# LingmaFuture/PRCV2025REID

Measured on AMD Instinct MI355X. Metric: multimodal instances/sec (PxK, 5-modality) at 1/2/4/8 GPU; eval queries/sec, higher is better.
Workload: dtype bf16; 1 GPU; P=16,K=4 per GPU, vis/nir/sk/cp 224x224 + text (T<=77), CLIP ViT-B/16 + text tower random-init, MER-LoRA r=8, masks all-on, 400 ids, SDM+CE, fwd+bwd+grad sanitise/clip+AdamW (reference default trainable set); P=16, K=4, global_batch=64, lora_rank=8, accum_steps=1, parallelism=dp1

## Files before the change

prcv2025reid_amd/csrc/attention.hip:

```cpp
#include "common.h"
#include <stdlib.h>

namespace {

typedef __attribute__((ext_vector_type(4))) short s4;
typedef __attribute__((address_space(3))) s4* lds_s4_ptr;

constexpr float LOG2E = 1.4426950408889634f;

__device__ __forceinline__ int swz(int row, int c) { return c ^ ((row >> 1) & 7); }

typedef const __attribute__((address_space(1))) void* gptr_t;
typedef __attribute__((address_space(3))) void* lptr_t;

template <int NT>
__device__ __forceinline__ void stage_head(const bf16_t* __restrict__ base, int ld, int S, char* lds, int wave, int lane,
                                           int row_limit = 1 << 30) {
#pragma unroll
    for (int i = 0; i < 4; ++i) {
        const int rblk = (i * NT + wave) * 8;
        if (rblk >= row_limit) continue;
        const int row = rblk + (lane >> 3);
        const int c = swz(row, lane & 7);
        const int grow = row < S ? row : S - 1;
        __builtin_amdgcn_global_load_lds((gptr_t)(base + (size_t)grow * ld + c * 8), (lptr_t)(lds + rblk * 128), 16, 0, 0);
    }
}

__device__ __forceinline__ bf16x8 row_frag(const char* img, int row0, int kchunk, int lane) {
    const int row = row0 + (lane & 31);
    return *(const bf16x8*)(img + row * 128 + (swz(row, kchunk + (lane >> 5)) << 4));
}

__device__ __forceinline__ bf16x8 col_frag(const char* img, int krow0, int col0, int lane) {
    const int h = lane >> 5, half16 = (lane >> 4) & 1, i = lane & 15;
    const int q = i >> 2, pp = i & 3;
    const int col = col0 + 16 * half16 + 4 * pp;
    const int r_lo = krow0 + 4 * h + q, r_hi = r_lo + 8;
    const char* a_lo = img + r_lo * 128 + (swz(r_lo, col >> 3) << 4) + (col & 7) * 2;
    const char* a_hi = img + r_hi * 128 + (swz(r_hi, col >> 3) << 4) + (col & 7) * 2;
    const s4 lo = __builtin_amdgcn_ds_read_tr16_b64_v4i16((lds_s4_ptr)a_lo);
    const s4 hi = __builtin_amdgcn_ds_read_tr16_b64_v4i16((lds_s4_ptr)a_hi);
    return bf16x8{lo[0], lo[1], lo[2], lo[3], hi[0], hi[1], hi[2], hi[3]};
}

__device__ __forceinline__ bf16x8 gfrag(const bf16_t* __restrict__ base, int ld, int row, int kchunk, int lane) {
    return *(const bf16x8*)(base + (size_t)row * ld + (kchunk + (lane >> 5)) * 8);
}

struct FragOff {
    int row[4];
    int col_lo[2];
    int col_hi[2];
};
__device__ __forceinline__ FragOff make_frag_off(int lane) {
    FragOff f;
    const int r = lane & 31, h = lane >> 5;
#pragma unroll
    for (int ks = 0; ks < 4; ++ks) f.row[ks] = r * 128 + (swz(r, 2 * ks + h) << 4);
    const int half16 = (lane >> 4) & 1, i = lane & 15, q = i >> 2, pp = i & 3;
    const int r_lo = 4 * h + q, r_hi = r_lo + 8;
#pragma unroll
    for (int dt = 0; dt < 2; ++dt) {
        const int col = dt * 32 + 16 * half16 + 4 * pp;
        f.col_lo[dt] = r_lo * 128 + (swz(r_lo, col >> 3) << 4) + (col & 7) * 2;
        f.col_hi[dt] = r_hi * 128 + (swz(r_hi, col >> 3) << 4) + (col & 7) * 2;
    }
    return f;
}
__device__ __forceinline__ bf16x8 row_frag_o(const char* img, int tile_row0, int ks, const FragOff& f) {
    return *(const bf16x8*)(img + tile_row0 * 128 + f.row[ks]);
}
__device__ __forceinline__ bf16x8 col_frag_o(const char* img, int krow0, int dt, const FragOff& f) {
    const s4 lo = __builtin_amdgcn_ds_read_tr16_b64_v4i16((lds_s4_ptr)(img + krow0 * 128 + f.col_lo[dt]));
    const s4 hi = __builtin_amdgcn_ds_read_tr16_b64_v4i16((lds_s4_ptr)(img + krow0 * 128 + f.col_hi[dt]));
    return bf16x8{lo[0], lo[1], lo[2], lo[3], hi[0], hi[1], hi[2], hi[3]};
}
__device__ __forceinline__ float fast_exp2(float x) { return __builtin_amdgcn_exp2f(x); }

__device__ __forceinline__ bf16x8 pack8(const f32x16& a, int s) {
    bf16x8 r;
#pragma unroll
    for (int j = 0; j < 8; ++j) r[j] = (short)f32_to_bf16(a[8 * s + j]);
    return r;
}

__device__ __forceinline__ int acc_row(int reg, int lane) { return (reg & 3) + 8 * (reg >> 2) + 4 * (lane >> 5); }

struct AttnParams {
    const bf16_t* qkv; int ld; const uint8_t* key_mask;
    bf16_t* out; int ldo; float* lse;
    const bf16_t* dout; bf16_t* dqkv; int lddqkv; float* delta;
    int n_seq, S, heads, causal;
    int q_tiles;
};

__device__ __forceinline__ void store_tile_row16(bf16_t* row, bool ok, const f32x16& t, float scale, int lane) {
#pragma unroll
    for (int j = 0; j < 2; ++j) {
        const int a = 8 * j, b = 8 * j + 4;
        const auto r0 = __builtin_amdgcn_permlane32_swap(pack_bf16x2(t[a] * scale, t[a + 1] * scale),
                                                         pack_bf16x2(t[b] * scale, t[b + 1] * scale), false, false);
        const auto r1 = __builtin_amdgcn_permlane32_swap(pack_bf16x2(t[a + 2] * scale, t[a + 3] * scale),
                                                         pack_bf16x2(t[b + 2] * scale, t[b + 3] * scale), false, false);
        if (ok) *(uint4*)(row + 8 * (2 * j + (lane >> 5))) = uint4{r0[0], r1[0], r0[1], r1[1]};
    }
}


template <int NT, bool TWO_PASS>
__global__ __launch_bounds__(NT * 64, TWO_PASS ? 4 : 1) void attn_fwd_kernel(const AttnParams p) {
    REID_T16_ENTER();
    extern __shared__ __attribute__((aligned(16))) char smem[];
    char* Ks = smem;
    char* Vs = smem + NT * 32 * 128;
    const int tid = threadIdx.x, lane = tid & 63;
    const int wave = __builtin_amdgcn_readfirstlane(tid >> 6);
    const int seq = blockIdx.x / p.heads, head = blockIdx.x % p.heads;
    const int d = p.heads * 64;
    const bf16_t* qb = p.qkv + (size_t)seq * p.S * p.ld + head * 64;
    stage_head<NT>(qb + d, p.ld, p.S, Ks, wave, lane);
    const int q0 = wave * 32;
    const int qi = q0 + (lane & 31);
    const int qrow = qi < p.S ? qi : p.S - 1;
    bf16x8 qf[4];
#pragma unroll
    for (int ks = 0; ks < 4; ++ks) qf[ks] = gfrag(qb, p.ld, qrow, 2 * ks, lane);
    stage_head<NT>(qb + 2 * d, p.ld, p.S, Vs, wave, lane);
    __syncthreads();
    if (q0 >= p.S || (p.q_tiles > 0 && wave >= p.q_tiles)) return;

    const FragOff fo = make_frag_off(lane);
    const uint8_t* km = p.key_mask ? p.key_mask + (size_t)seq * p.S : nullptr;
    const int h4 = 4 * (lane >> 5);
    const bool general = km != nullptr || p.causal;
    auto score_tile = [&](int kt) -> f32x16 {
        f32x16 t;
#pragma unroll
        for (int e = 0; e < 16; ++e) t[e] = 0.f;
#pragma unroll
        for (int ks = 0; ks < 4; ++ks) t = mfma32(row_frag_o(Ks, kt * 32, ks, fo), qf[ks], t);
        if (general) {
#pragma unroll
            for (int e = 0; e < 16; ++e) {
                const int key = kt * 32 + (e & 3) + 8 * (e >> 2) + h4;
                bool ok = key < p.S;
                if (ok && km) ok = km[key] != 0;
                if (p.causal) ok = ok && key <= qi;
                t[e] = ok ? t[e] : -INFINITY;
            }
        } else if (kt == NT - 1) {
#pragma unroll
            for (int e = 0; e < 16; ++e) {
                const int key = kt * 32 + (e & 3) + 8 * (e >> 2) + h4;
                t[e] = key < p.S ? t[e] : -INFINITY;
            }
        }
        return t;
    };
    const float c = 0.125f * LOG2E;
    f32x16 ot[2];
#pragma unroll
    for (int dt = 0; dt < 2; ++dt)
#pragma unroll
        for (int e = 0; e < 16; ++e) ot[dt][e] = 0.f;
    float mx = -INFINITY, l = 0.f;
    if (TWO_PASS) {
#pragma unroll 1
        for (int kt = 0; kt < NT; ++kt) {
            const f32x16 t = score_tile(kt);
#pragma unroll
            for (int e = 0; e < 16; e += 2) mx = fmaxf(mx, fmaxf(t[e], t[e + 1]));
        }
        mx = fmaxf(mx, __shfl_xor(mx, 32, 64));
        if (mx == -INFINITY) mx = 0.f;
        const float nmc = -mx * c;
#pragma unroll 1
        for (int kt = 0; kt < NT; ++kt) {
            f32x16 t = score_tile(kt);
#pragma unroll
            for (int e = 0; e < 16; ++e) {
                const float pe = fast_exp2(fmaf(t[e], c, nmc));
                t[e] = pe;
                l += pe;
            }
#pragma unroll
            for (int s2 = 0; s2 < 2; ++s2) {
                const bf16x8 pf = pack8(t, s2);
#pragma unroll
                for (int dt = 0; dt < 2; ++dt) ot[dt] = mfma32(col_frag_o(Vs, kt * 32 + 16 * s2, dt, fo), pf, ot[dt]);
            }
        }
    } else {
        f32x16 st[NT];
#pragma unroll
        for (int kt = 0; kt < NT; ++kt) st[kt] = score_tile(kt);
#pragma unroll
        for (int kt = 0; kt < NT; ++kt)
#pragma unroll
            for (int e = 0; e < 16; e += 2) mx = fmaxf(mx, fmaxf(st[kt][e], st[kt][e + 1]));
        mx = fmaxf(mx, __shfl_xor(mx, 32, 64));
        if (mx == -INFINITY) mx = 0.f;
        const float nmc = -mx * c;
#pragma unroll
        for (int kt = 0; kt < NT; ++kt)
#pragma unroll
            for (int e = 0; e < 16; ++e) {
                const float pe = fast_exp2(fmaf(st[kt][e], c, nmc));
                st[kt][e] = pe;
                l += pe;
            }
#pragma unroll
        for (int kt = 0; kt < NT; ++kt)
#pragma unroll
            for (int s2 = 0; s2 < 2; ++s2) {
                const bf16x8 pf = pack8(st[kt], s2);
#pragma unroll
                for (int dt = 0; dt < 2; ++dt) ot[dt] = mfma32(col_frag_o(Vs, kt * 32 + 16 * s2, dt, fo), pf, ot[dt]);
            }
    }
    l += __shfl_xor(l, 32, 64);
    {
        const float inv = 1.0f / l;
        bf16_t* orow = p.out + ((size_t)seq * p.S + qrow) * p.ldo + head * 64;
#pragma unroll
        for (int dt = 0; dt < 2; ++dt) store_tile_row16(orow + dt * 32, qi < p.S, ot[dt], inv, lane);
        if (qi < p.S && p.lse && lane < 32) p.lse[((size_t)seq * p.heads + head) * p.S + qi] = mx * 0.125f + logf(l);
    }
}

template <int NT>
__global__ __launch_bounds__(NT * 64) void attn_bwd_dkv_kernel(const AttnParams p) {
    REID_T16_ENTER();
    extern __shared__ __attribute__((aligned(16))) char smem[];
    char* Qs = smem;
    char* Gs = smem + NT * 32 * 128;
    float* rowc = (float*)(smem + 2 * NT * 32 * 128);
    const int tid = threadIdx.x, lane = tid & 63;
    const int wave = __builtin_amdgcn_readfirstlane(tid >> 6);
    const int seq = blockIdx.x / p.heads, head = blockIdx.x % p.heads;
    const int d = p.heads * 64;
    const bf16_t* qb = p.qkv + (size_t)seq * p.S * p.ld + head * 64;
    const bf16_t* gb = p.dout + (size_t)seq * p.S * p.ldo + head * 64;
    const int q_rows = p.q_tiles > 0 ? p.q_tiles * 32 : NT * 32;
    stage_head<NT>(qb, p.ld, p.S, Qs, wave, lane, q_rows);
    stage_head<NT>(gb, p.ldo, p.S, Gs, wave, lane, q_rows);
    for (int t = tid; t < NT * 32; t += NT * 64) {
        const size_t o = ((size_t)seq * p.heads + head) * p.S + t;
        rowc[t] = t < p.S ? -p.lse[o] * LOG2E : -INFINITY;
        rowc[NT * 32 + t] = t < p.S ? -p.delta[o] * 0.125f : 0.f;
    }
    const int k0 = wave * 32;
    const int ki = k0 + (lane & 31);
    const int krow = ki < p.S ? ki : p.S - 1;
    bf16x8 kf[4], vf[4];
#pragma unroll
    for (int ks = 0; ks < 4; ++ks) {
        kf[ks] = gfrag(qb + d, p.ld, krow, 2 * ks, lane);
        vf[ks] = gfrag(qb + 2 * d, p.ld, krow, 2 * ks, lane);
    }
    __syncthreads();
    if (k0 >= p.S) return;
    const uint8_t* km = p.key_mask ? p.key_mask + (size_t)seq * p.S : nullptr;
    const bool key_ok = ki < p.S && (!km || km[ki] != 0);

    const FragOff fo = make_frag_off(lane);
    f32x16 dkt[2], dvt[2];
#pragma unroll
    for (int dt = 0; dt < 2; ++dt)
#pragma unroll
        for (int e = 0; e < 16; ++e) { dkt[dt][e] = 0.f; dvt[dt][e] = 0.f; }
    const float c = 0.125f * LOG2E;
    const int h4 = 4 * (lane >> 5);
    for (int qt = 0; qt < NT; ++qt) {
        if (qt * 32 >= p.S || (p.q_tiles > 0 && qt >= p.q_tiles)) break;
        f32x16 s, dp;
#pragma unroll
        for (int e = 0; e < 16; ++e) { s[e] = 0.f; dp[e] = 0.f; }
#pragma unroll
        for (int ks = 0; ks < 4; ++ks) {
            s = mfma32(row_frag_o(Qs, qt * 32, ks, fo), kf[ks], s);
            dp = mfma32(row_frag_o(Gs, qt * 32, ks, fo), vf[ks], dp);
        }
        f32x16 pm, ds;
#pragma unroll
        for (int g = 0; g < 4; ++g) {
            const f32x4 nl = *(const f32x4*)(rowc + qt * 32 + 8 * g + h4);
            const f32x4 nd = *(const f32x4*)(rowc + NT * 32 + qt * 32 + 8 * g + h4);
#pragma unroll
            for (int j = 0; j < 4; ++j) {
                const int e = 4 * g + j;
                float pe = fast_exp2(fmaf(s[e], c, nl[j]));
                if (p.causal && ki > qt * 32 + 8 * g + h4 + j) pe = 0.f;
                pm[e] = pe;
                ds[e] = pe * fmaf(dp[e], 0.125f, nd[j]);
            }
        }
#pragma unroll
        for (int s2 = 0; s2 < 2; ++s2) {
            const bf16x8 pf = pack8(pm, s2), df = pack8(ds, s2);
#pragma unroll
            for (int dt = 0; dt < 2; ++dt) {
                dvt[dt] = mfma32(col_frag_o(Gs, qt * 32 + 16 * s2, dt, fo), pf, dvt[dt]);
                dkt[dt] = mfma32(col_frag_o(Qs, qt * 32 + 16 * s2, dt, fo), df, dkt[dt]);
            }
        }
    }
    if (!key_ok) {
#pragma unroll
        for (int dt = 0; dt < 2; ++dt)
#pragma unroll
            for (int e = 0; e < 16; ++e) { dkt[dt][e] = 0.f; dvt[dt][e] = 0.f; }
    }
    {
        const bool ok = ki < p.S;
        bf16_t* drow = p.dqkv + ((size_t)seq * p.S + (ok ? ki : 0)) * p.lddqkv + head * 64;
#pragma unroll
        for (int dt = 0; dt < 2; ++dt) {
            store_tile_row16(drow + d + dt * 32, ok, dkt[dt], 1.0f, lane);
            store_tile_row16(drow + 2 * d + dt * 32, ok, dvt[dt], 1.0f, lane);
        }
    }
}

template <int NT>
__global__ __launch_bounds__(NT * 64) void attn_bwd_dq_kernel(const AttnParams p) {
    REID_T16_ENTER();
    extern __shared__ __attribute__((aligned(16))) char smem[];
    char* Ks = smem;
    char* Vs = smem + NT * 32 * 128;
    const int tid = threadIdx.x, lane = tid & 63;
    const int wave = __builtin_amdgcn_readfirstlane(tid >> 6);
    const int seq = blockIdx.x / p.heads, head = blockIdx.x % p.heads;
    const int d = p.heads * 64;
    const bf16_t* qb = p.qkv + (size_t)seq * p.S * p.ld + head * 64;
    const bf16_t* gb = p.dout + (size_t)seq * p.S * p.ldo + head * 64;
    stage_head<NT>(qb + d, p.ld, p.S, Ks, wave, lane);
    stage_head<NT>(qb + 2 * d, p.ld, p.S, Vs, wave, lane);
    const int q0 = wave * 32;
    const int qi = q0 + (lane & 31);
    const int qrow = qi < p.S ? qi : p.S - 1;
    bf16x8 qf[4], gf[4];
#pragma unroll
    for (int ks = 0; ks < 4; ++ks) {
        qf[ks] = gfrag(qb, p.ld, qrow, 2 * ks, lane);
        gf[ks] = gfrag(gb, p.ldo, qrow, 2 * ks, lane);
    }
    const size_t so = ((size_t)seq * p.heads + head) * p.S + qrow;
    const float nl = -p.lse[so] * LOG2E;
    float dsum = 0.f;
    {
        const bf16_t* ob = p.out + (size_t)seq * p.S * p.ldo + head * 64;
#pragma unroll
        for (int ks = 0; ks < 4; ++ks) {
            const bf16x8 of = gfrag(ob, p.ldo, qrow, 2 * ks, lane);
#pragma unroll
            for (int j = 0; j < 8; ++j) dsum = fmaf(bf16_to_f32((bf16_t)gf[ks][j]), bf16_to_f32((bf16_t)of[j]), dsum);
        }
    }
    dsum += __shfl_xor(dsum, 32, 64);
    if (qi < p.S && lane < 32) p.delta[so] = dsum;
    const float nd = -dsum * 0.125f;
    __syncthreads();
    if (q0 >= p.S) return;
    if (p.q_tiles > 0 && wave >= p.q_tiles) {
        if (qi < p.S) {
            bf16_t* drow = p.dqkv + ((size_t)seq * p.S + qi) * p.lddqkv + head * 64;
#pragma unroll
            for (int dt = 0; dt < 2; ++dt)
#pragma unroll
                for (int g = 0; g < 4; ++g) *(uint2*)(drow + dt * 32 + 8 * g + 4 * (lane >> 5)) = uint2{0u, 0u};
        }
        return;
    }
    const uint8_t* km = p.key_mask ? p.key_mask + (size_t)seq * p.S : nullptr;
    const FragOff fo = make_frag_off(lane);
    f32x16 dqt[2];
#pragma unroll
    for (int dt = 0; dt < 2; ++dt)
#pragma unroll
        for (int e = 0; e < 16; ++e) dqt[dt][e] = 0.f;
    const float c = 0.125f * LOG2E;
    const int h4 = 4 * (lane >> 5);
    const bool slow = km != nullptr || p.causal;
    for (int kt = 0; kt < NT; ++kt) {
        if (kt * 32 >= p.S) break;
        f32x16 s, dp;
#pragma unroll
        for (int e = 0; e < 16; ++e) { s[e] = 0.f; dp[e] = 0.f; }
#pragma unroll
        for (int ks = 0; ks < 4; ++ks) {
            s = mfma32(row_frag_o(Ks, kt * 32, ks, fo), qf[ks], s);
            dp = mfma32(row_frag_o(Vs, kt * 32, ks, fo), gf[ks], dp);
        }
        const bool edge = slow || (kt + 1) * 32 > p.S;
        f32x16 ds;
#pragma unroll
        for (int e = 0; e < 16; ++e) {
            float pe = fast_exp2(fmaf(s[e], c, nl));
            if (edge) {
                const int key = kt * 32 + (e & 3) + 8 * (e >> 2) + h4;
                bool ok = key < p.S;
                if (ok && km) ok = km[key] != 0;
                if (p.causal) ok = ok && key <= qi;
                pe = ok ? pe : 0.f;
            }
            ds[e] = pe * fmaf(dp[e], 0.125f, nd);
        }
#pragma unroll
        for (int s2 = 0; s2 < 2; ++s2) {
            const bf16x8 df = pack8(ds, s2);
#pragma unroll
            for (int dt = 0; dt < 2; ++dt) dqt[dt] = mfma32(col_frag_o(Ks, kt * 32 + 16 * s2, dt, fo), df, dqt[dt]);
        }
    }
    {
        const bool ok = qi < p.S;
        bf16_t* drow = p.dqkv + ((size_t)seq * p.S + (ok ? qi : 0)) * p.lddqkv + head * 64;
#pragma unroll
        for (int dt = 0; dt < 2; ++dt) store_tile_row16(drow + dt * 32, ok, dqt[dt], 1.0f, lane);
    }
}

__device__ __forceinline__ int ds_chunk(int r, int c) { return c ^ ((r >> 1) & 3); }
#ifdef REID_ATTN_TRACE
__device__ unsigned long long* g_attn_bwd_trace = nullptr;
#define ATTN_BWD_STAMP(slot) do { if (g_attn_bwd_trace && threadIdx.x == 0) g_attn_bwd_trace[(size_t)blockIdx.x * 8 + (slot)] = __builtin_amdgcn_s_memrealtime(); } while (0)
#else
#define ATTN_BWD_STAMP(slot) do { } while (0)
#endif
template <int NT>
__global__ __launch_bounds__(NT * 64) void attn_bwd_fused_kernel(const AttnParams p) {
    REID_T16_ENTER();
    ATTN_BWD_STAMP(0);
    extern __shared__ __attribute__((aligned(16))) char smem[];
    constexpr int IMG = NT * 32 * 128;
    constexpr int DS_ROW = NT * 64;
    char* Qs = smem;
    char* Gs = smem + IMG;
    char* Ks = smem;
    char* Ds = smem + 2 * IMG;
    float* rowc = (float*)(Ds + NT * 32 * DS_ROW);
    const int tid = threadIdx.x, lane = tid & 63;
    const int wave = __builtin_amdgcn_readfirstlane(tid >> 6);
    const int seq = blockIdx.x / p.heads, head = blockIdx.x % p.heads;
    const int d = p.heads * 64;
    const bf16_t* qb = p.qkv + (size_t)seq * p.S * p.ld + head * 64;
    const bf16_t* gb = p.dout + (size_t)seq * p.S * p.ldo + head * 64;
    const bf16_t* ob = p.out + (size_t)seq * p.S * p.ldo + head * 64;
    const int nq = p.q_tiles > 0 ? (p.q_tiles < NT ? p.q_tiles : NT) : NT;
    const int q_rows = nq * 32;
    const int t0 = wave * 32;
    const int ti = t0 + (lane & 31);
    const int trow = ti < p.S ? ti : p.S - 1;
    const bool own_q = wave < nq;
    bf16x8 kf[4], vf[4];
#pragma unroll
    for (int ks = 0; ks < 4; ++ks) {
        kf[ks] = gfrag(qb + d, p.ld, trow, 2 * ks, lane);
        vf[ks] = gfrag(qb + 2 * d, p.ld, trow, 2 * ks, lane);
    }
    stage_head<NT>(qb, p.ld, p.S, Qs, wave, lane, q_rows);
    stage_head<NT>(gb, p.ldo, p.S, Gs, wave, lane, q_rows);
    bf16x8 of[4];
#pragma unroll
    for (int ks = 0; ks < 4; ++ks) of[ks] = gfrag(ob, p.ldo, trow, 2 * ks, lane);
    const size_t so = ((size_t)seq * p.heads + head) * p.S + trow;
    const float lse_v = p.lse[so];
    const FragOff fo = make_frag_off(lane);
    __syncthreads();
    ATTN_BWD_STAMP(1);
    {
        float dsum = 0.f;
        if (own_q) {
#pragma unroll
            for (int ks = 0; ks < 4; ++ks) {
                const bf16x8 gfk = row_frag_o(Gs, t0, ks, fo);
#pragma unroll
                for (int j = 0; j < 8; ++j) dsum = fmaf(bf16_to_f32((bf16_t)gfk[j]), bf16_to_f32((bf16_t)of[ks][j]), dsum);
            }
        }
        dsum += __shfl_xor(dsum, 32, 64);
        if (lane < 32) {
            const bool live = own_q && ti < p.S;
            rowc[ti] = live ? -lse_v * LOG2E : -INFINITY;
            rowc[NT * 32 + ti] = live ? -dsum * 0.125f : 0.f;
            if (live && p.delta) p.delta[so] = dsum;
        }
    }
    __syncthreads();
    ATTN_BWD_STAMP(2);
    const float c = 0.125f * LOG2E;
    const int h4 = 4 * (lane >> 5);
    const bool tile_ok = ti < p.S;
    bf16_t* trow_out = p.dqkv + ((size_t)seq * p.S + trow) * p.lddqkv + head * 64;

    {
        f32x16 dkt[2], dvt[2];
#pragma unroll
        for (int dt = 0; dt < 2; ++dt)
#pragma unroll
            for (int e = 0; e < 16; ++e) { dkt[dt][e] = 0.f; dvt[dt][e] = 0.f; }
        const int hsw = (lane >> 5) ^ (((lane & 31) >> 1) & 3);
        char* const ds_w0 = Ds + ti * DS_ROW + 16 * hsw;
        char* const ds_w1 = Ds + ti * DS_ROW + 16 * (hsw ^ 2);
        const int nqt = nq < (p.S + 31) / 32 ? nq : (p.S + 31) / 32;
        auto scores = [&](int qt, f32x16& s, f32x16& dp) {
#pragma unroll
            for (int e = 0; e < 16; ++e) { s[e] = 0.f; dp[e] = 0.f; }
#pragma unroll
            for (int ks = 0; ks < 4; ++ks) {
                s = mfma32(row_frag_o(Qs, qt * 32, ks, fo), kf[ks], s);
                dp = mfma32(row_frag_o(Gs, qt * 32, ks, fo), vf[ks], dp);
            }
        };
        f32x16 s, dp, s_n, dp_n;
        if (nqt > 0) scores(0, s, dp);
        for (int qt = 0; qt < nqt; ++qt) {
            if (qt + 1 < nqt) scores(qt + 1, s_n, dp_n);
#pragma unroll
            for (int s2 = 0; s2 < 2; ++s2) {
                bf16x8 pf, df;
#pragma unroll
                for (int g2 = 0; g2 < 2; ++g2) {
                    const int g = 2 * s2 + g2;
                    const f32x4 nl = *(const f32x4*)(rowc + qt * 32 + 8 * g + h4);
                    const f32x4 nd = *(const f32x4*)(rowc + NT * 32 + qt * 32 + 8 * g + h4);
#pragma unroll
                    for (int j = 0; j < 4; ++j) {
                        const int e = 4 * g + j;
                        const float pe = fast_exp2(fmaf(s[e], c, nl[j]));
                        pf[4 * g2 + j] = (short)f32_to_bf16(pe);
                        df[4 * g2 + j] = (short)f32_to_bf16(pe * fmaf(dp[e], 0.125f, nd[j]));
                    }
                }
#pragma unroll
                for (int dt = 0; dt < 2; ++dt) {
                    dvt[dt] = mfma32(col_frag_o(Gs, qt * 32 + 16 * s2, dt, fo), pf, dvt[dt]);
                    dkt[dt] = mfma32(col_frag_o(Qs, qt * 32 + 16 * s2, dt, fo), df, dkt[dt]);
                }
                *(bf16x8*)((s2 ? ds_w1 : ds_w0) + qt * 64) = tile_ok ? df : bf16x8{};
            }
            s = s_n; dp = dp_n;
        }
        ATTN_BWD_STAMP(3);
#pragma unroll
        for (int dt = 0; dt < 2; ++dt) {
            store_tile_row16(trow_out + d + dt * 32, tile_ok, dkt[dt], 1.0f, lane);
            store_tile_row16(trow_out + 2 * d + dt * 32, tile_ok, dvt[dt], 1.0f, lane);
        }
    }

    __syncthreads();
#pragma unroll
    for (int ks = 0; ks < 4; ++ks) *(bf16x8*)(Ks + t0 * 128 + fo.row[ks]) = kf[ks];
    __syncthreads();
    ATTN_BWD_STAMP(4);

    if (!own_q) {
        if (tile_ok) {
#pragma unroll
            for (int dt = 0; dt < 2; ++dt)
#pragma unroll
                for (int g = 0; g < 4; ++g) *(uint2*)(trow_out + dt * 32 + 8 * g + 4 * (lane >> 5)) = uint2{0u, 0u};
        }
        return;
    }
    {
        const int h = lane >> 5, half16 = (lane >> 4) & 1, q = (lane & 15) >> 2, pp = lane & 3;
        const int r = 4 * h + q;
        const int ds_r = r * DS_ROW + 16 * ds_chunk(r, 4 * wave + 2 * half16 + (pp & 1)) + 8 * (pp >> 1);
        f32x16 dqt[2];
#pragma unroll
        for (int dt = 0; dt < 2; ++dt)
#pragma unroll
            for (int e = 0; e < 16; ++e) dqt[dt][e] = 0.f;
#pragma unroll
        for (int kt = 0; kt < NT; ++kt)
#pragma unroll
            for (int s2 = 0; s2 < 2; ++s2) {
                const int krow0 = kt * 32 + 16 * s2;
                const s4 lo = __builtin_amdgcn_ds_read_tr16_b64_v4i16((lds_s4_ptr)(Ds + krow0 * DS_ROW + ds_r));
                const s4 hi = __builtin_amdgcn_ds_read_tr16_b64_v4i16((lds_s4_ptr)(Ds + (krow0 + 8) * DS_ROW + ds_r));
                const bf16x8 df = bf16x8{lo[0], lo[1], lo[2], lo[3], hi[0], hi[1], hi[2], hi[3]};
#pragma unroll
                for (int dt = 0; dt < 2; ++dt) dqt[dt] = mfma32(col_frag_o(Ks, krow0, dt, fo), df, dqt[dt]);
            }
        ATTN_BWD_STAMP(5);
#pragma unroll
        for (int dt = 0; dt < 2; ++dt) store_tile_row16(trow_out + dt * 32, tile_ok, dqt[dt], 1.0f, lane);
        ATTN_BWD_STAMP(6);
    }
}

template <int NT>
int launch_fwd(const AttnParams& p, hipStream_t s) {
    constexpr int LDS = 2 * NT * 32 * 128;
    constexpr bool TP = NT >= 4;
    REID_MAX_LDS((attn_fwd_kernel<NT, TP>), LDS);
    hipLaunchKernelGGL((attn_fwd_kernel<NT, TP>), dim3(p.n_seq * p.heads), dim3(NT * 64), LDS, s, p);
    REID_CHECK_LAUNCH("reid_attn_fwd");
    return REID_OK;
}

template <int NT>
int launch_bwd(const AttnParams& p, hipStream_t s) {
    constexpr int LDS1 = 2 * NT * 32 * 128 + 2 * NT * 32 * 4;
    constexpr int LDS2 = 2 * NT * 32 * 128;
    REID_MAX_LDS((attn_bwd_dkv_kernel<NT>), LDS1);
    REID_MAX_LDS((attn_bwd_dq_kernel<NT>), LDS2);
    if (!p.key_mask && !p.causal && reid_knob(KNOB_ATTN_BWD) != 1) {
        constexpr int LDSF = 2 * NT * 32 * 128 + (NT * 32) * (NT * 64) + 2 * NT * 32 * 4;
        REID_MAX_LDS((attn_bwd_fused_kernel<NT>), LDSF);
        hipLaunchKernelGGL(attn_bwd_fused_kernel<NT>, dim3(p.n_seq * p.heads), dim3(NT * 64), LDSF, s, p);
        REID_CHECK_LAUNCH("reid_attn_bwd(fused)");
        return REID_OK;
    }
    hipLaunchKernelGGL(attn_bwd_dq_kernel<NT>, dim3(p.n_seq * p.heads), dim3(NT * 64), LDS2, s, p);
    REID_CHECK_LAUNCH("reid_attn_bwd(dq)");
    hipLaunchKernelGGL(attn_bwd_dkv_kernel<NT>, dim3(p.n_seq * p.heads), dim3(NT * 64), LDS1, s, p);
    REID_CHECK_LAUNCH("reid_attn_bwd(dkv)");
    return REID_OK;
}

int check_common(const char* name, const void* qkv, int ld, int n_seq, int S, int heads) {
    REID_CHECK_ARG(qkv != nullptr, "%s: null qkv", name);
    REID_CHECK_ARG(n_seq > 0 && heads > 0 && S > 0 && S <= 224, "%s: S=%d must be in 1..224 (n_seq=%d heads=%d)", name, S, n_seq, heads);
    REID_CHECK_ARG(ld >= 3 * heads * 64 && ld % 8 == 0, "%s: ld=%d must be >= 3*heads*64 and a multiple of 8", name, ld);
    return REID_OK;
}

}

#ifdef REID_ATTN_TRACE
extern "C" void reid_debug_attn_bwd_trace(void* buf) {
    unsigned long long* ptr = (unsigned long long*)buf;
    (void)hipMemcpyToSymbol(HIP_SYMBOL(g_attn_bwd_trace), &ptr, sizeof(ptr));
}
#endif

#define DISPATCH_NT(nt, fn, ...)                \
    switch (nt) {                               \
        case 1: return fn<1>(__VA_ARGS__);      \
        case 2: return fn<2>(__VA_ARGS__);      \
        case 3: return fn<3>(__VA_ARGS__);      \
        case 4: return fn<4>(__VA_ARGS__);      \
        case 5: return fn<5>(__VA_ARGS__);      \
        case 6: return fn<6>(__VA_ARGS__);      \
        default: return fn<7>(__VA_ARGS__);     \
    }

extern "C" int reid_attn_fwd(const void* qkv, int32_t ld, const uint8_t* key_mask, void* out, int32_t ldo, float* lse,
                             int32_t n_seq, int32_t S, int32_t heads, int32_t causal, int32_t q_tiles, void* stream) {
    int rc = check_common("reid_attn_fwd", qkv, ld, n_seq, S, heads);
    if (rc) return rc;
    REID_CHECK_ARG(out && ldo >= heads * 64 && ldo % 4 == 0, "reid_attn_fwd: out/ldo");
    AttnParams p{(const bf16_t*)qkv, ld, key_mask, (bf16_t*)out, ldo, lse, nullptr, nullptr, 0, nullptr, n_seq, S, heads, causal, q_tiles};
    DISPATCH_NT((S + 31) / 32, launch_fwd, p, (hipStream_t)stream)
}

extern "C" int reid_attn_bwd(const void* qkv, int32_t ld, const uint8_t* key_mask, const void* out, const void* dout,
                             int32_t ldo, const float* lse, void* dqkv, int32_t lddqkv, float* delta_ws, int32_t n_seq,
                             int32_t S, int32_t heads, int32_t causal, int32_t q_tiles, void* stream) {
    int rc = check_common("reid_attn_bwd", qkv, ld, n_seq, S, heads);
    if (rc) return rc;
    REID_CHECK_ARG(out && dout && lse && dqkv && delta_ws, "reid_attn_bwd: null pointer");
    REID_CHECK_ARG(ldo >= heads * 64 && ldo % 8 == 0 && lddqkv >= 3 * heads * 64 && lddqkv % 4 == 0, "reid_attn_bwd: ldo/lddqkv");
    AttnParams p{(const bf16_t*)qkv, ld, key_mask, (bf16_t*)out, ldo, (float*)lse, (const bf16_t*)dout, (bf16_t*)dqkv, lddqkv,
                 delta_ws, n_seq, S, heads, causal, q_tiles};
    DISPATCH_NT((S + 31) / 32, launch_bwd, p, (hipStream_t)stream)
}
```

prcv2025reid_amd/csrc/common.h:

```cpp
#pragma once
#include <hip/hip_runtime.h>
#include <stdint.h>
#include <stdio.h>
#include "../../include/reid_hip.h"

typedef __attribute__((ext_vector_type(8))) short bf16x8;
typedef __attribute__((ext_vector_type(4))) short bf16x4;
typedef __attribute__((ext_vector_type(4))) float f32x4;
typedef __attribute__((ext_vector_type(16))) float f32x16;
typedef unsigned short bf16_t;

__attribute__((visibility("hidden"))) void reid_set_error(const char* fmt, ...);

enum reid_knob_id { KNOB_GEMM_TILE, KNOB_ATTN_BWD, KNOB_LORA_IMPL, KNOB_LN_IMPL, KNOB_TOPK_TILE, KNOB_TOPK_SCAN, KNOB_COUNT };
__attribute__((visibility("hidden"))) int reid_knob(int id);
__attribute__((visibility("hidden"))) int reid_num_cus();

#define REID_CHECK_ARG(cond, ...)                     \
    do {                                              \
        if (!(cond)) {                                \
            reid_set_error(__VA_ARGS__);              \
            return REID_ERR_ARG;                      \
        }                                             \
    } while (0)

static inline hipError_t reid_max_dyn_lds(const void* fn, int bytes, unsigned* done_mask) {
    int dev = 0;
    hipError_t e = hipGetDevice(&dev);
    if (e != hipSuccess) return e;
    if (dev >= 0 && dev < 32 && ((__atomic_load_n(done_mask, __ATOMIC_ACQUIRE) >> dev) & 1u)) return hipSuccess;
    e = hipFuncSetAttribute(fn, hipFuncAttributeMaxDynamicSharedMemorySize, bytes);
    if (e == hipSuccess && dev >= 0 && dev < 32) __atomic_fetch_or(done_mask, 1u << dev, __ATOMIC_RELEASE);
    return e;
}
#define REID_MAX_LDS(kernel, bytes)                                                                              \
    do {                                                                                                         \
        static unsigned lds_done_ = 0;                                                                           \
        const hipError_t le_ = reid_max_dyn_lds((const void*)(kernel), (int)(bytes), &lds_done_);                \
        if (le_ != hipSuccess) {                                                                                 \
            reid_set_error("hipFuncSetAttribute(%s, dynamic LDS %d): %s", #kernel, (int)(bytes), hipGetErrorString(le_)); \
            return REID_ERR_LAUNCH;                                                                              \
        }                                                                                                        \
    } while (0)

#define REID_CHECK_HIP(call, what)                                                     \
    do {                                                                               \
        const hipError_t he_ = (call);                                                 \
        if (he_ != hipSuccess) {                                                       \
            reid_set_error("%s: %s", what, hipGetErrorString(he_));                    \
            return REID_ERR_LAUNCH;                                                    \
        }                                                                              \
    } while (0)

#define REID_CHECK_LAUNCH(name)                                                        \
    do {                                                                               \
        hipError_t e_ = hipGetLastError();                                             \
        if (e_ != hipSuccess) {                                                        \
            reid_set_error("%s: launch failed: %s", name, hipGetErrorString(e_));     \
            return REID_ERR_LAUNCH;                                                    \
        }                                                                              \
    } while (0)

typedef _Float16 __attribute__((ext_vector_type(8))) half8_t;
#ifdef REID_FLAVOR_F16
__device__ __forceinline__ float bf16_to_f32(bf16_t v) { return (float)__builtin_bit_cast(_Float16, v); }
__device__ __forceinline__ bf16_t f32_to_bf16(float f) { return __builtin_bit_cast(bf16_t, (_Float16)f); }
__device__ __forceinline__ f32x4 mfma16(bf16x8 a, bf16x8 b, f32x4 c) {
    return __builtin_amdgcn_mfma_f32_16x16x32_f16(__builtin_bit_cast(half8_t, a), __builtin_bit_cast(half8_t, b), c, 0, 0, 0);
}
__device__ __forceinline__ f32x16 mfma32(bf16x8 a, bf16x8 b, f32x16 c) {
    return __builtin_amdgcn_mfma_f32_32x32x16_f16(__builtin_bit_cast(half8_t, a), __builtin_bit_cast(half8_t, b), c, 0, 0, 0);
}
#define REID_T16_ENTER() __builtin_amdgcn_s_setreg(1 | (23 << 6) | (0 << 11), 1)
#define REID_FLAVOR_ID 1
#define REID_T16_EPS 0.0009765625f
#else
__device__ __forceinline__ float bf16_to_f32(bf16_t v) { return __uint_as_float(((uint32_t)v) << 16); }
__device__ __forceinline__ bf16_t f32_to_bf16(float f) {
    __bf16 b = (__bf16)f;
    return __builtin_bit_cast(bf16_t, b);
}
__device__ __forceinline__ f32x4 mfma16(bf16x8 a, bf16x8 b, f32x4 c) { return __builtin_amdgcn_mfma_f32_16x16x32_bf16(a, b, c, 0, 0, 0); }
__device__ __forceinline__ f32x16 mfma32(bf16x8 a, bf16x8 b, f32x16 c) { return __builtin_amdgcn_mfma_f32_32x32x16_bf16(a, b, c, 0, 0, 0); }
#define REID_T16_ENTER() do { } while (0)
#define REID_FLAVOR_ID 0
#define REID_T16_EPS 0.00390625f
#endif

typedef float pk_f32x2 __attribute__((ext_vector_type(2)));
#ifdef REID_FLAVOR_F16
typedef _Float16 pk_t16x2 __attribute__((ext_vector_type(2)));
#else
typedef __bf16 pk_t16x2 __attribute__((ext_vector_type(2)));
#endif
__device__ __forceinline__ uint32_t pack_bf16x2(float lo, float hi) {
    const pk_t16x2 r = __builtin_convertvector(pk_f32x2{lo, hi}, pk_t16x2);
    return __builtin_bit_cast(uint32_t, r);
}

typedef _Float16 pk_h16x2 __attribute__((ext_vector_type(2)));
__device__ __forceinline__ uint32_t pack_f16x2(float lo, float hi) {
    const pk_h16x2 r = __builtin_convertvector(pk_f32x2{lo, hi}, pk_h16x2);
    return __builtin_bit_cast(uint32_t, r);
}
__device__ __forceinline__ float f16_to_f32(unsigned short v) { return (float)__builtin_bit_cast(_Float16, v); }
#define REID_F16_SATURATE() __builtin_amdgcn_s_setreg(1 | (23 << 6) | (0 << 11), 1)
__device__ __forceinline__ bool f16_clamps(float v) { const float a = fabsf(v); return a >= 65520.f && a <= 3.402823466e38f; }

__device__ __forceinline__ float wave_sum(float v) {
#pragma unroll
    for (int o = 32; o > 0; o >>= 1) v += __shfl_xor(v, o, 64);
    return v;
}
__device__ __forceinline__ float wave_max(float v) {
#pragma unroll
    for (int o = 32; o > 0; o >>= 1) v = fmaxf(v, __shfl_xor(v, o, 64));
    return v;
}

__device__ __forceinline__ void gauss_cdf_pdf(float x, float& cdf, float& pdf_unnorm) {
    const float z = fabsf(x) * 0.70710678118654752f;
    const float t = __builtin_amdgcn_rcpf(fmaf(0.3275911f, z, 1.0f));
    const float e = __builtin_amdgcn_exp2f(x * x * -0.72134752044448170f);
    const float poly = t * fmaf(t, fmaf(t, fmaf(t, fmaf(t, 1.061405429f, -1.453152027f), 1.421413741f), -0.284496736f), 0.254829592f);
    const float q = 0.5f * poly * e;
    cdf = x >= 0.f ? 1.0f - q : q;
    pdf_unnorm = e;
}
__device__ __forceinline__ float gelu_erf_f(float x) {
    float c, e;
    gauss_cdf_pdf(x, c, e);
    return x * c;
}
__device__ __forceinline__ void gelu_both_f(float x, float& g, float& dg) {
    float c, e;
    gauss_cdf_pdf(x, c, e);
    g = x * c;
    dg = fmaf(x * 0.39894228040143268f, e, c);
}
typedef float f32x2_t __attribute__((ext_vector_type(2)));
__device__ __forceinline__ void gelu_both_x2(f32x2_t x, f32x2_t& g, f32x2_t& dg) {
    const f32x2_t xs = (x * x) * -0.72134752044448170f;
    f32x2_t e; e.x = __builtin_amdgcn_exp2f(xs.x); e.y = __builtin_amdgcn_exp2f(xs.y);
    f32x2_t z; z.x = __builtin_fabsf(x.x); z.y = __builtin_fabsf(x.y);
    const f32x2_t den = z * (0.3275911f * 0.70710678118654752f) + 1.0f;
    f32x2_t t; t.x = __builtin_amdgcn_rcpf(den.x); t.y = __builtin_amdgcn_rcpf(den.y);
    f32x2_t poly = t * (0.5f * 1.061405429f) + (0.5f * -1.453152027f);
    poly = poly * t + (0.5f * 1.421413741f);
    poly = poly * t + (0.5f * -0.284496736f);
    poly = poly * t + (0.5f * 0.254829592f);
    const f32x2_t q = (poly * t) * e;
    const f32x2_t h = 0.5f - q;
    f32x2_t sh; sh.x = __builtin_copysignf(h.x, x.x); sh.y = __builtin_copysignf(h.y, x.y);
    const f32x2_t cdf = sh + 0.5f;
    g = x * cdf;
    dg = (x * 0.39894228040143268f) * e + cdf;
}
__device__ __forceinline__ float dgelu_erf_f(float x) {
    float c, e;
    gauss_cdf_pdf(x, c, e);
    return fmaf(x * 0.39894228040143268f, e, c);
}
__device__ __forceinline__ float quick_gelu_f(float x) { return x / (1.0f + __expf(-1.702f * x)); }
__device__ __forceinline__ float dquick_gelu_f(float x) {
    const float s = 1.0f / (1.0f + __expf(-1.702f * x));
    return s + x * 1.702f * s * (1.0f - s);
}
```

prcv2025reid_amd/csrc/rowops.hip:

```cpp
#include "common.h"
#include <stdarg.h>
#include <string.h>
#include <stdlib.h>

static thread_local char g_err[512] = "";
void reid_set_error(const char* fmt, ...) {
    va_list ap;
    va_start(ap, fmt);
    vsnprintf(g_err, sizeof(g_err), fmt, ap);
    va_end(ap);
}
extern "C" const char* reid_last_error(void) { return g_err; }
extern "C" int reid_version(void) { return REID_ABI_VERSION; }

static const char* const g_knob_names[] = {"GEMM_TILE", "ATTN_BWD", "LORA_IMPL", "LN_IMPL", "TOPK_TILE", "TOPK_SCAN"};
static_assert(sizeof(g_knob_names) / sizeof(g_knob_names[0]) == KNOB_COUNT, "one name per reid_knob_id");
static int g_knobs[KNOB_COUNT];
static int* knob_table() {
    static const bool init = [] {
        for (int i = 0; i < KNOB_COUNT; ++i) {
            char name[64];
            snprintf(name, sizeof(name), "REID_%s", g_knob_names[i]);
            const char* e = getenv(name);
            g_knobs[i] = e ? atoi(e) : -1;
        }
        return true;
    }();
    (void)init;
    return g_knobs;
}
int reid_knob(int id) { return knob_table()[id]; }
extern "C" int reid_set_knob(const char* name, int value) {
    int* t = knob_table();
    for (int i = 0; i < KNOB_COUNT; ++i)
        if (strcmp(name, g_knob_names[i]) == 0) {
            t[i] = value; return REID_OK;
        }
    reid_set_error("reid_set_knob: unknown knob %s", name);
    return REID_ERR_ARG;
}
int reid_num_cus() {
    static const int n = [] {
        int dev = 0;
        hipDeviceProp_t prop;
        if (hipGetDevice(&dev) != hipSuccess || hipGetDeviceProperties(&prop, dev) != hipSuccess) return 256;
        return prop.multiProcessorCount > 0 ? prop.multiProcessorCount : 256;
    }();
    return n;
}
extern "C" int reid_flavor(void) { return REID_FLAVOR_ID; }
extern "C" int reid_check_device(int dev) {
    hipDeviceProp_t prop;
    if (hipGetDeviceProperties(&prop, dev) != hipSuccess) {
        reid_set_error("reid_check_device: hipGetDeviceProperties(%d) failed", dev);
        return REID_ERR_DEVICE;
    }
    if (strncmp(prop.gcnArchName, "gfx950", 6) != 0) {
        reid_set_error("reid_check_device: device %d is %s, this library is built for gfx950 only", dev, prop.gcnArchName);
        return REID_ERR_DEVICE;
    }
    return REID_OK;
}

namespace {

constexpr int MAXV = 4;

__global__ __launch_bounds__(256) void ln_fwd_kernel(const float* __restrict__ x, int ldx, const int32_t* __restrict__ row_index,
                                                     const float* __restrict__ gamma, const float* __restrict__ beta,
                                                     bf16_t* __restrict__ yb, float* __restrict__ yf, int ldy,
                                                     float* __restrict__ mean, float* __restrict__ rstd, int rows,
                                                     int cols, float eps) {
    REID_T16_ENTER();
    const int lane = threadIdx.x & 63;
    const int row = blockIdx.x * 4 + (threadIdx.x >> 6);
    if (row >= rows) return;
    const size_t src = row_index ? (size_t)row_index[row] : (size_t)row;
    const float* xr = x + src * ldx;
    const int nv = cols >> 2;
    f32x4 v[MAXV];
    float s = 0.f;
#pragma unroll
    for (int i = 0; i < MAXV; ++i) {
        const int c = lane + i * 64;
        v[i] = c < nv ? *(const f32x4*)(xr + c * 4) : f32x4{0.f, 0.f, 0.f, 0.f};
        s += v[i][0] + v[i][1] + v[i][2] + v[i][3];
    }
    const float mu = wave_sum(s) / cols;
    float q = 0.f;
#pragma unroll
    for (int i = 0; i < MAXV; ++i) {
        const int c = lane + i * 64;
        if (c < nv) {
#pragma unroll
            for (int e = 0; e < 4; ++e) { const float d = v[i][e] - mu; q += d * d; }
        }
    }
    const float rs = rsqrtf(wave_sum(q) / cols + eps);
    if (lane == 0) {
        if (mean) mean[row] = mu;
        if (rstd) rstd[row] = rs;
    }
#pragma unroll
    for (int i = 0; i < MAXV; ++i) {
        const int c = lane + i * 64;
        if (c < nv) {
            const f32x4 g = *(const f32x4*)(gamma + c * 4);
            const f32x4 b = *(const f32x4*)(beta + c * 4);
            f32x4 o;
#pragma unroll
            for (int e = 0; e < 4; ++e) o[e] = (v[i][e] - mu) * rs * g[e] + b[e];
            if (yf) *(f32x4*)(yf + (size_t)row * ldy + c * 4) = o;
            if (yb) *(uint2*)(yb + (size_t)row * ldy + c * 4) = uint2{pack_bf16x2(o[0], o[1]), pack_bf16x2(o[2], o[3])};
        }
    }
}

template <bool Y_HALF>
__global__ __launch_bounds__(256) void add_ln_fwd_kernel(const float* __restrict__ x, int ldx, const bf16_t* __restrict__ y, int ldy,
                                                         const float* __restrict__ row_scale, int rows_per_img,
                                                         float* __restrict__ xo, int ldxo, const float* __restrict__ gamma,
                                                         const float* __restrict__ beta, bf16_t* __restrict__ hb, int ldh,
                                                         float* __restrict__ mean, float* __restrict__ rstd, int rows, int cols, float eps) {
    REID_T16_ENTER();
    const int lane = threadIdx.x & 63;
    const int row = blockIdx.x * 4 + (threadIdx.x >> 6);
    if (row >= rows) return;
    const float* xr = x + (size_t)row * ldx;
    const bf16_t* yr = y + (size_t)row * ldy;
    const float sc = row_scale ? row_scale[row / rows_per_img] : 1.f;
    const int nv = cols >> 2;
    f32x4 v[MAXV];
    float s = 0.f;
#pragma unroll
    for (int i = 0; i < MAXV; ++i) {
        const int c = lane + i * 64;
        if (c < nv) {
            const f32x4 a = *(const f32x4*)(xr + c * 4);
            const bf16x4 b = *(const bf16x4*)(yr + c * 4);
#pragma unroll
            for (int e = 0; e < 4; ++e) v[i][e] = fmaf(sc, Y_HALF ? f16_to_f32((unsigned short)b[e]) : bf16_to_f32((bf16_t)b[e]), a[e]);
            *(f32x4*)(xo + (size_t)row * ldxo + c * 4) = v[i];
        } else {
            v[i] = f32x4{0.f, 0.f, 0.f, 0.f};
        }
        s += v[i][0] + v[i][1] + v[i][2] + v[i][3];
    }
    const float mu = wave_sum(s) / cols;
    float q = 0.f;
#pragma unroll
    for (int i = 0; i < MAXV; ++i) {
        const int c = lane + i * 64;
        if (c < nv) {
#pragma unroll
            for (int e = 0; e < 4; ++e) { const float d = v[i][e] - mu; q += d * d; }
        }
    }
    const float rs = rsqrtf(wave_sum(q) / cols + eps);
    if (lane == 0) {
        if (mean) mean[row] = mu;
        if (rstd) rstd[row] = rs;
    }
#pragma unroll
    for (int i = 0; i < MAXV; ++i) {
        const int c = lane + i * 64;
        if (c < nv) {
            const f32x4 g = *(const f32x4*)(gamma + c * 4);
            const f32x4 b = *(const f32x4*)(beta + c * 4);
            f32x4 o;
#pragma unroll
            for (int e = 0; e < 4; ++e) o[e] = (v[i][e] - mu) * rs * g[e] + b[e];
            *(uint2*)(hb + (size_t)row * ldh + c * 4) = uint2{pack_bf16x2(o[0], o[1]), pack_bf16x2(o[2], o[3])};
        }
    }
}

template <bool DY_BF16, bool AFFINE, bool DX_HALF, int VN = MAXV>
__global__ __launch_bounds__(256) void ln_bwd_kernel(const void* __restrict__ dy, int lddy, const float* __restrict__ x, int ldx,
                                                     const int32_t* __restrict__ row_index, const float* __restrict__ gamma,
                                                     const float* __restrict__ mean, const float* __restrict__ rstd,
                                                     const void* __restrict__ dres_, void* __restrict__ dx_,
                                                     bf16_t* __restrict__ dxb, int lddx, float* __restrict__ dgamma,
                                                     float* __restrict__ dbeta, int rows, int cols,
                                                     const float* __restrict__ bscale, int rows_per_img, int* __restrict__ overflow) {
    REID_T16_ENTER();
    if (DX_HALF) REID_F16_SATURATE();
    const int lane = threadIdx.x & 63;
    const int nv = cols >> 2;
    constexpr bool affine = AFFINE;
    f32x4 ag[VN], ab[VN];
#pragma unroll
    for (int i = 0; i < VN; ++i) { ag[i] = f32x4{0.f, 0.f, 0.f, 0.f}; ab[i] = ag[i]; }
    for (int row = blockIdx.x * 4 + (threadIdx.x >> 6); row < rows; row += gridDim.x * 4) {
        const size_t xrow = row_index ? (size_t)row_index[row] : (size_t)row;
        const float* xr = x + xrow * ldx;
        const float mu = mean[row], rs = rstd[row];
        f32x4 xh[VN], g[VN];
        float s1 = 0.f, s2 = 0.f;
#pragma unroll
        for (int i = 0; i < VN; ++i) {
            const int c = lane + i * 64;
            xh[i] = f32x4{0.f, 0.f, 0.f, 0.f}; g[i] = xh[i];
            if (c < nv) {
                const f32x4 xv = *(const f32x4*)(xr + c * 4);
                const f32x4 gm = *(const f32x4*)(gamma + c * 4);
                f32x4 d;
                if (DY_BF16) {
                    const bf16x4 t = *(const bf16x4*)((const bf16_t*)dy + (size_t)row * lddy + c * 4);
#pragma unroll
                    for (int e = 0; e < 4; ++e) d[e] = bf16_to_f32((bf16_t)t[e]);
                } else {
                    d = *(const f32x4*)((const float*)dy + (size_t)row * lddy + c * 4);
                }
#pragma unroll
                for (int e = 0; e < 4; ++e) {
                    xh[i][e] = (xv[e] - mu) * rs;
                    if (affine) { ag[i][e] = fmaf(d[e], xh[i][e], ag[i][e]); ab[i][e] += d[e]; }
                    g[i][e] = d[e] * gm[e];
                    s1 += g[i][e];
                    s2 += g[i][e] * xh[i][e];
                }
            }
        }
        const float m1 = wave_sum(s1) / cols, m2 = wave_sum(s2) / cols;
        const float bs = bscale ? bscale[xrow / rows_per_img] : 1.f;
        bool clamped = false;
#pragma unroll
        for (int i = 0; i < VN; ++i) {
            const int c = lane + i * 64;
            if (c < nv) {
                f32x4 o;
#pragma unroll
                for (int e = 0; e < 4; ++e) o[e] = rs * (g[i][e] - m1 - xh[i][e] * m2);
                if (DX_HALF) {
                    if (dres_) {
                        const uint2 r = *(const uint2*)((const unsigned short*)dres_ + xrow * lddx + c * 4);
                        o[0] += f16_to_f32((unsigned short)(r.x & 0xffffu)); o[1] += f16_to_f32((unsigned short)(r.x >> 16));
                        o[2] += f16_to_f32((unsigned short)(r.y & 0xffffu)); o[3] += f16_to_f32((unsigned short)(r.y >> 16));
                    }
#pragma unroll
                    for (int e = 0; e < 4; ++e) clamped |= f16_clamps(o[e]) || (REID_FLAVOR_ID == 1 && dxb && f16_clamps(o[e] * bs));
                    *(uint2*)((unsigned short*)dx_ + xrow * lddx + c * 4) = uint2{pack_f16x2(o[0], o[1]), pack_f16x2(o[2], o[3])};
                } else {
                    if (dres_) {
                        const f32x4 r = *(const f32x4*)((const float*)dres_ + xrow * lddx + c * 4);
                        o += r;
                    }
                    *(f32x4*)((float*)dx_ + xrow * lddx + c * 4) = o;
                }
                if (dxb) *(uint2*)(dxb + xrow * lddx + c * 4) = uint2{pack_bf16x2(o[0] * bs, o[1] * bs), pack_bf16x2(o[2] * bs, o[3] * bs)};
            }
        }
        if (DX_HALF && overflow && __ballot(clamped) && lane == 0) atomicOr(overflow, 1);
    }
    if (affine) {
#pragma unroll
        for (int i = 0; i < VN; ++i) {
            const int c = lane + i * 64;
            if (c < nv) {
#pragma unroll
                for (int e = 0; e < 4; ++e) {
                    if (dgamma) atomicAdd(dgamma + c * 4 + e, ag[i][e]);
                    if (dbeta) atomicAdd(dbeta + c * 4 + e, ab[i][e]);
                }
            }
        }
    }
}

__global__ __launch_bounds__(256) void im2col_kernel(const float* __restrict__ img, bf16_t* __restrict__ out, int n_img, int H,
                                                     int W, int P, int cin) {
    REID_T16_ENTER();
    const int gw = W / P, gh = H / P;
    const int kc = cin * P * P;
    const int chunks_per_row = kc / 8;
    const long total = (long)n_img * gh * gw * chunks_per_row;
    for (long i = (long)blockIdx.x * blockDim.x + threadIdx.x; i < total; i += (long)gridDim.x * blockDim.x) {
        const int ch = i % chunks_per_row;
        const long prow = i / chunks_per_row;
        const int pw = prow % gw, ph = (prow / gw) % gh;
        const long b = prow / (gw * gh);
        const int k = ch * 8;
        const int c = k / (P * P), py = (k / P) % P, px = k % P;
        const size_t base = ((size_t)b * 3) * H * W + (size_t)(ph * P + py) * W + pw * P + px;
        float v[8];
        if (cin == 3) {
            const float* s = img + base + (size_t)c * H * W;
            const f32x4 a = *(const f32x4*)s, bb = *(const f32x4*)(s + 4);
#pragma unroll
            for (int e = 0; e < 4; ++e) { v[e] = a[e]; v[4 + e] = bb[e]; }
        } else {
#pragma unroll
            for (int e = 0; e < 8; ++e) v[e] = 0.f;
            for (int cc = 0; cc < 3; ++cc) {
                const float* s = img + base + (size_t)cc * H * W;
                const f32x4 a = *(const f32x4*)s, bb = *(const f32x4*)(s + 4);
#pragma unroll
                for (int e = 0; e < 4; ++e) { v[e] += a[e]; v[4 + e] += bb[e]; }
            }
#pragma unroll
            for (int e = 0; e < 8; ++e) v[e] = v[e] / 3.0f;
        }
        uint4 o = {pack_bf16x2(v[0], v[1]), pack_bf16x2(v[2], v[3]), pack_bf16x2(v[4], v[5]), pack_bf16x2(v[6], v[7])};
        *(uint4*)(out + (size_t)prow * kc + k) = o;
    }
}

__global__ void cls_rows_kernel(const float* __restrict__ cls, const float* __restrict__ pos0, float* __restrict__ x, int ldx,
                                int n_img, int tokens, int cols) {
    REID_T16_ENTER();
    const int i = blockIdx.x * blockDim.x + threadIdx.x;
    const int nv = cols >> 2;
    if (i >= n_img * nv) return;
    const int b = i / nv, c = i % nv;
    const f32x4 a = *(const f32x4*)(cls + c * 4), p = *(const f32x4*)(pos0 + c * 4);
    *(f32x4*)(x + (size_t)b * tokens * ldx + c * 4) = a + p;
}

// ... 312 lines not shown
```

Measured before the change: 2148 instances/s.

## Replace two-sweep attention forward softmax with single-pass online softmax

For sequences with four or more key tiles, the forward attention kernel now computes each score tile once and applies an online softmax. It tracks a running max, rescales the accumulators only when a wave-wide ballot shows the max grew, and software-pipelines the next tile's score MMA ahead of the current tile's exp and PV. This removes the second QK^T sweep that the previous two-pass scheme recomputed, and it skips key tiles past the true sequence length. The old two-sweep path remains behind a new ATTN_FWD knob. The costs are occasional rescale work, higher register pressure from holding two score tiles, and a shifted knob enum order.

```diff
diff --git a/prcv2025reid_amd/csrc/attention.hip b/prcv2025reid_amd/csrc/attention.hip
--- a/prcv2025reid_amd/csrc/attention.hip
+++ b/prcv2025reid_amd/csrc/attention.hip
@@ -108,8 +108,8 @@
 }
 
 
-template <int NT, bool TWO_PASS>
-__global__ __launch_bounds__(NT * 64, TWO_PASS ? 4 : 1) void attn_fwd_kernel(const AttnParams p) {
+template <int NT, bool STREAM, bool TWO_SWEEP>
+__global__ __launch_bounds__(NT * 64, STREAM ? 4 : 1) void attn_fwd_kernel(const AttnParams p) {
     REID_T16_ENTER();
     extern __shared__ __attribute__((aligned(16))) char smem[];
     char* Ks = smem;
@@ -165,7 +165,50 @@
 #pragma unroll
         for (int e = 0; e < 16; ++e) ot[dt][e] = 0.f;
     float mx = -INFINITY, l = 0.f;
-    if (TWO_PASS) {
+    if (STREAM && !TWO_SWEEP) {
+        auto absorb = [&](f32x16& t, int kt) {
+            float tm = fmaxf(t[0], t[1]);
+#pragma unroll
+            for (int e = 2; e < 16; e += 2) tm = fmaxf(tm, fmaxf(t[e], t[e + 1]));
+            tm = fmaxf(tm, __shfl_xor(tm, 32, 64));
+            const float mn = fmaxf(mx, tm);
+            if (__builtin_amdgcn_ballot_w64(mn > mx) != 0) {
+                const float a = mx == -INFINITY ? 0.f : fast_exp2((mx - mn) * c);
+#pragma unroll
+                for (int dt = 0; dt < 2; ++dt)
+#pragma unroll
+                    for (int e = 0; e < 16; ++e) ot[dt][e] *= a;
+                l *= a;
+                mx = mn;
+            }
+            const float nmc = mx == -INFINITY ? 0.f : -mx * c;
+#pragma unroll
+            for (int e = 0; e < 16; ++e) {
+                const float pe = fast_exp2(fmaf(t[e], c, nmc));
+                t[e] = pe;
+                l += pe;
+            }
+#pragma unroll
+            for (int s2 = 0; s2 < 2; ++s2) {
+                if (kt * 32 + 16 * s2 >= p.S) break;
+                const bf16x8 pf = pack8(t, s2);
+#pragma unroll
+                for (int dt = 0; dt < 2; ++dt) ot[dt] = mfma32(col_frag_o(Vs, kt * 32 + 16 * s2, dt, fo), pf, ot[dt]);
+            }
+        };
+        const int nt = __builtin_amdgcn_readfirstlane((p.S + 31) >> 5);
+        f32x16 ta = score_tile(0), tb;
+#pragma unroll 1
+        for (int kt = 0; kt < nt; kt += 2) {
+            if (kt + 1 < nt) tb = score_tile(kt + 1);
+            absorb(ta, kt);
+            if (kt + 1 < nt) {
+                if (kt + 2 < nt) ta = score_tile(kt + 2);
+                absorb(tb, kt + 1);
+            }
+        }
+        if (mx == -INFINITY) mx = 0.f;
+    } else if (STREAM) {
 #pragma unroll 1
         for (int kt = 0; kt < NT; ++kt) {
             const f32x16 t = score_tile(kt);
@@ -596,9 +639,14 @@
 template <int NT>
 int launch_fwd(const AttnParams& p, hipStream_t s) {
     constexpr int LDS = 2 * NT * 32 * 128;
-    constexpr bool TP = NT >= 4;
-    REID_MAX_LDS((attn_fwd_kernel<NT, TP>), LDS);
-    hipLaunchKernelGGL((attn_fwd_kernel<NT, TP>), dim3(p.n_seq * p.heads), dim3(NT * 64), LDS, s, p);
+    constexpr bool STREAM = NT >= 4;
+    if (STREAM && reid_knob(KNOB_ATTN_FWD) == 1) {
+        REID_MAX_LDS((attn_fwd_kernel<NT, STREAM, STREAM>), LDS);
+        hipLaunchKernelGGL((attn_fwd_kernel<NT, STREAM, STREAM>), dim3(p.n_seq * p.heads), dim3(NT * 64), LDS, s, p);
+    } else {
+        REID_MAX_LDS((attn_fwd_kernel<NT, STREAM, false>), LDS);
+        hipLaunchKernelGGL((attn_fwd_kernel<NT, STREAM, false>), dim3(p.n_seq * p.heads), dim3(NT * 64), LDS, s, p);
+    }
     REID_CHECK_LAUNCH("reid_attn_fwd");
     return REID_OK;
 }
diff --git a/prcv2025reid_amd/csrc/common.h b/prcv2025reid_amd/csrc/common.h
--- a/prcv2025reid_amd/csrc/common.h
+++ b/prcv2025reid_amd/csrc/common.h
@@ -12,7 +12,7 @@
 
 __attribute__((visibility("hidden"))) void reid_set_error(const char* fmt, ...);
 
-enum reid_knob_id { KNOB_GEMM_TILE, KNOB_ATTN_BWD, KNOB_LORA_IMPL, KNOB_LN_IMPL, KNOB_TOPK_TILE, KNOB_TOPK_SCAN, KNOB_COUNT };
+enum reid_knob_id { KNOB_GEMM_TILE, KNOB_ATTN_BWD, KNOB_ATTN_FWD, KNOB_LORA_IMPL, KNOB_LN_IMPL, KNOB_TOPK_TILE, KNOB_TOPK_SCAN, KNOB_COUNT };
 __attribute__((visibility("hidden"))) int reid_knob(int id);
 __attribute__((visibility("hidden"))) int reid_num_cus();
 
diff --git a/prcv2025reid_amd/csrc/rowops.hip b/prcv2025reid_amd/csrc/rowops.hip
--- a/prcv2025reid_amd/csrc/rowops.hip
+++ b/prcv2025reid_amd/csrc/rowops.hip
@@ -13,7 +13,7 @@
 extern "C" const char* reid_last_error(void) { return g_err; }
 extern "C" int reid_version(void) { return REID_ABI_VERSION; }
 
-static const char* const g_knob_names[] = {"GEMM_TILE", "ATTN_BWD", "LORA_IMPL", "LN_IMPL", "TOPK_TILE", "TOPK_SCAN"};
+static const char* const g_knob_names[] = {"GEMM_TILE", "ATTN_BWD", "ATTN_FWD", "LORA_IMPL", "LN_IMPL", "TOPK_TILE", "TOPK_SCAN"};
 static_assert(sizeof(g_knob_names) / sizeof(g_knob_names[0]) == KNOB_COUNT, "one name per reid_knob_id");
 static int g_knobs[KNOB_COUNT];
 static int* knob_table() {
```

Result: no change. 2155 instances/s, median of 6 (+0.3%).
